# VITA-Group/CV_A-FAN

Measured on AMD Instinct MI355X. Metric: images/sec (whole node) A-FAN K=5 train step, ResNet-18/CIFAR-10, higher is better.
Workload: dtype bf16; 1 GPU; resnet18 CIFAR-10-shape A-FAN K=5 bf16, batch 256/GPU, perturb_idx 6, internal layout nhwc, 1xMI355X per rank (BASELINE configs[1]); global_batch=256, parallelism=dp1, hipgraph=True, in_launch_batchnorm=True

## Files before the change

### cv_a-fan_amd/_lib.py

```python
import ctypes as C
import os

_HERE = os.path.dirname(os.path.abspath(__file__))
LIB_PATH = os.environ.get("AFAN_HIP_LIB") or os.path.join(_HERE, "libafan_hip.so")

AFAN_F32, AFAN_BF16 = 0, 1
AFAN_NCHW, AFAN_NHWC = 0, 1
_ERRORS = {-1: "AFAN_EDTYPE (unknown dtype code)", -2: "AFAN_EALIGN (misaligned pointer)",
           -3: "AFAN_ESHAPE (bad sizes)", -4: "AFAN_ENULL (required pointer is NULL)",
           -5: "AFAN_ELAYOUT (unknown layout code)"}

_p, _i, _l, _f = C.c_void_p, C.c_int, C.c_int64, C.c_float

SIGNATURES = {
    "afan_version": (_i, []),
    "afan_arch": (C.c_char_p, []),
    "afan_pgd_step": (_i, [_p, _p, _i, _p, _p, _l, _f, _f, _i, _p]),
    "afan_tensor_clamp": (_i, [_p, _p, _p, _l, _p]),
    "afan_norms_workspace_floats": (_l, [_l, _l]),
    "afan_pgd_step_norms": (_i, [_p, _p, _i, _p, _p, _l, _l, _f, _f, _i, _p, _p, _p, _p]),
    "afan_perturb_norms": (_i, [_p, _p, _l, _l, _p, _p, _p, _p]),
    "afan_axpy_noise": (_i, [_p, _p, _l, _f, _p, _p]),
    "afan_mix_feature": (_i, [_p, _p, _p, _l, _l, _l, _f, _i, _p]),
    "afan_mix_feature_nhwc": (_i, [_p, _p, _p, _l, _l, _l, _f, _i, _p]),
    "afan_lerp_points": (_i, [_p, _p, _p, _l, C.POINTER(_f), _i, _p]),
    "afan_lerp_mix": (_i, [_p, _p, _p, _l, _l, _l, C.POINTER(_f), _i, C.c_uint, _f, _i, _p]),
    "afan_head_max_classes": (_i, []),
    "afan_head_forward": (_i, [_p, _i, _l, _l, _l, _p, _p, _l, _p, _p, _p]),
    "afan_head_backward": (_i, [_p, _p, _p, _l, _l, _l, _l, _p, _i, _p, _p, _i, _p]),
    "afan_cross_entropy": (_i, [_p, _p, _l, _l, _p, _p, _p]),
    "afan_mix_w_workspace_floats": (_l, []),
    "afan_mix_w": (_i, [_p, _p, _p, _p, _i, _l, _p]),
    "afan_mix_w_backward": (_i, [_p, _i, _p, _p, _l, _p, _p, _i, _p]),
    "afan_bn_workspace_floats": (_l, [_l]),
    "afan_bn_acc_doubles": (_l, [_l]),
    "afan_bn_acc_supported": (_i, [_i, _l]),
    "afan_bn_set_running_updates": (_i, [_i]),
    "afan_bn_running_update": (_i, [_p, _l, C.c_double, _f, _f, _p, _p, _p, _p]),
    "afan_bn_running_update_batched": (_i, [_p, _p, _p, _p, _p, _p, _p, _p, _i, _p]),
    "afan_bn_train_forward_acc": (_i, [_p, _p, _p, _i, _l, _l, _l, _f, _f, _p, _p, _i, _p, _i, _p, _p, _p, _p, _i, _p]),
    "afan_bn_train_forward_acc_dual": (_i, [_p, _p, _p, _i, _l, _l, _l, _f, _f, _p, _p, _p, _p, _p, _p, _p, _f, _f, _p, _p, _p, _p,
                                            _p, _p, _p, _p]),
    "afan_bn_backward_acc": (_i, [_p, _p, _p, _p, _p, _i, _l, _l, _l, _p, _i, _p, _i, _p, _p, _i, _i, _p]),
    "afan_bn_stats": (_i, [_p, _i, _i, _l, _l, _l, _f, _f, _p, _p, _p, _p, _p, _p]),
    "afan_bn_train_forward": (_i, [_p, _p, _p, _i, _i, _l, _l, _l, _f, _f, _p, _p, _i, _p, _p, _p, _p, _p, _p]),
    "afan_bn_apply": (_i, [_p, _p, _p, _i, _i, _l, _l, _l, _p, _p, _p, _p, _i, _p, _p]),
    "afan_bn_backward": (_i, [_p, _p, _p, _p, _p, _i, _i, _l, _l, _l, _p, _p, _p, _i, _p, _p, _p, _i, _p, _l, _p]),
    "afan_conv_supported": (_i, [_l, _l, _i, _i]),
    "afan_conv_fwd_nhwc_bf16": (_i, [_p, _p, _p, _l, _l, _l, _l, _l, _i, _i, _i, _p, _p, _p, _i, _p]),
    "afan_conv_fwd_affine_nhwc_bf16": (_i, [_p, _p, _p, _l, _l, _l, _l, _l, _i, _i, _p, _p, _i, _p]),
    "afan_conv_fwd_affine_any_nhwc_bf16": (_i, [_p, _p, _p, _l, _l, _l, _l, _l, _i, _i, _p, _p, _i, _p]),
    "afan_conv_fwd_multi_nhwc_bf16": (_i, [_p, _p, _p, _i, _l, _l, _l, _l, _l, _p, _i, _p, _p, _p, _i, _p]),
    "afan_conv_fwd_tiles": (_l, [_l, _l, _l, _l, _l, _i, _i]),
# ... 79 lines not shown
    "afan_proposal_rows": (_i, [_p, _l, _p, _l, _p, _l, _p, _p, _p]),
    "afan_labels_limit": (_i, [_p, _l, _l, _p, _l, _p]),
    "afan_det_loss_bwd": (_i, [_p, _p, _p, _p, _p, _p, _l, _l, _l, _l, _l, _p, _p, _p]),
    "afan_roi_align_fwd": (_i, [_p, _p, _p, _i, _i, _l, _l, _l, _l, _i, _i, _f, _i, _p]),
    "afan_roi_align_bwd": (_i, [_p, _p, _p, _i, _i, _l, _l, _l, _l, _l, _i, _i, _f, _i, _p]),
    "afan_roi_align_bwd_workspace_bytes": (_l, [_l, _l, _l]),
    "afan_roi_align_bwd_ws": (_i, [_p, _p, _p, _i, _i, _l, _l, _l, _l, _l, _i, _i, _f, _i, _p, _p]),
    "afan_transpose_weights": (_i, [_p, _p, _p, _i, _l, _p]),
    "afan_sgd_step": (_i, [_p, _p, _p, _p, _l, _p, _f, _f, _f, _i, _p]),
    "afan_sgd_step_guarded": (_i, [_p, _p, _p, _p, _l, _p, _f, _f, _f, _i, _p, _p]),
    "afan_guarded_copy": (_i, [_p, _p, _l, _p, _p, _p]),
    "afan_occupy_cus": (_i, [_i, _i, _i, _p]),
    "afan_cast_bf16": (_i, [_p, _p, _l, _p]),
    "afan_pgd_init": (_i, [_p, _i, _p, _p, _p, _l, _p]),
    "afan_normalize_nchw": (_i, [_p, _p, _i, _i, _l, _l, _l, _p, _p, _p]),
    "afan_profile_enable": (_i, [_i]),
    "afan_profile_collect": (_i, [C.c_char_p, C.POINTER(_l), C.POINTER(C.c_double), C.POINTER(C.c_double),
                                  C.POINTER(C.c_double), _i]),
    "afan_profile_event_overhead": (_i, [_i, C.POINTER(_f), _p]),
    "afan_conv_trace": (_i, [_i]),
    "afan_conv_trace_read": (_i, [C.POINTER(_l), C.c_char_p, _i]),
}

_lib = None


class AfanLibraryError(RuntimeError):
    pass


def load():
    global _lib
    if _lib is not None:
        return _lib
    if not os.path.exists(LIB_PATH):
        raise AfanLibraryError(
            f"{LIB_PATH} is missing: build it with `python -c 'import __graft_entry__ as g; g.build()'` "
            "(or `make -C cv_a-fan_amd/csrc`). There is no CPU or PyTorch fallback for the A-FAN kernels.")
    lib = C.CDLL(LIB_PATH)
    for name, (res, args) in SIGNATURES.items():
        fn = getattr(lib, name)
        fn.restype = res
        fn.argtypes = args
    _lib = lib
    return lib


def check(rc, what):
    if rc == 0:
        return
    if rc < 0:
        raise AfanLibraryError(f"{what}: {_ERRORS.get(rc, rc)}")
    raise AfanLibraryError(f"{what}: HIP launch failed with hipError_t={rc}")
```

### cv_a-fan_amd/attack_algo.py

```python
import torch

from . import ops
from .resnet_s import _dense, _like_layout, dgrad_only, fused_criterion

__all__ = ["PGD", "tensor_clamp", "linfball_proj", "mix_feature", "get_sample_points", "last_norms"]

_last = {"l2": None, "linf": None}


def last_norms():
    return _last["l2"], _last["linf"]


def tensor_clamp(t, min, max, in_place=True):
    res = t if in_place else t.clone()
    ops.tensor_clamp_(res.data, min.contiguous(), max.contiguous())
    return res


def linfball_proj(center, radius, t, in_place=True):
    res = t if in_place else t.clone()
    zero = torch.zeros_like(res.data)
    ops.pgd_step_(res.data, zero, 0.0, x_clean=center.contiguous(), eps=float(radius), clip=True)
    return res


def PGD(x, loss_fn, y=None, model=None, steps=3, gamma=None, start_idx=1, layer_number=16, eps=(2 / 255),
        randinit=False, clip=False, with_norms=False, grad0=None):
    if x.device.type != "cuda":
        raise ops.AfanLibraryError("PGD: x must live on the MI355X (no CPU path in this build)")
    lp = getattr(model, "compute_dtype", torch.float32) == torch.bfloat16
    if grad0 is not None and (randinit or steps < 1):
        raise ValueError("grad0 is the gradient at x: not with randinit, and only when there is a first step")
    x, x_adv, shadow = ops.pgd_init(_dense(x.detach()), want_shadow=lp and grad0 is None and not randinit)
    if lp and shadow is None:
        shadow = torch.empty_like(x, dtype=torch.bfloat16)
    if randinit:
        u = _like_layout(torch.rand(x_adv.shape).to(x.device, non_blocking=True), x_adv)
        ops.axpy_noise_(x_adv, u, eps, shadow)
    l2 = linf = None
    loss_fn = fused_criterion(loss_fn, model)
    for t in range(steps):
        if t == 0 and grad0 is not None:
            grad = grad0.detach()
        else:
            xin = (shadow if lp else x_adv).detach().requires_grad_(True)
            with dgrad_only():
                out = model(xin, end_point=layer_number, start_point=start_idx)
                loss = loss_fn(out, y)
                root = ops.one(loss.device) if (loss.dim() == 0 and loss.dtype == torch.float32) else None
                grad = torch.autograd.grad(loss, xin, grad_outputs=root, only_inputs=True)[0]
        grad = _like_layout(grad, x_adv)
        if with_norms and t == steps - 1:
            l2, linf = ops.pgd_step_norms_(x_adv, grad, gamma, x, eps, clip, shadow)
        else:
            ops.pgd_step_(x_adv, grad, gamma, x, eps, clip, shadow)
    if with_norms:
        if l2 is None:
            l2, linf = ops.perturb_norms(x_adv, x)
        _last["l2"], _last["linf"] = l2, linf
    x_adv.requires_grad_(True)
    if lp:
        x_adv._afan_shadow = shadow
    return x_adv


def mix_feature(clean_feature, adv_feature):
    return ops.mix_feature(_dense(clean_feature), _dense(adv_feature), 1e-5)


# ... 14 lines not shown
```

### cv_a-fan_amd/csrc/afan_bn_nhwc.hip

```cpp
#include "afan_common.h"
#include <stdlib.h>

using namespace afan;

namespace afan_nhwc {

constexpr int BLOCK = 256;
constexpr int MAX_G = 512;

template <typename T, int VEC> struct LdV {
    __device__ static __forceinline__ void ld(const T* p, float (&v)[VEC]) {
        if constexpr (VEC == 1) v[0] = Elt<T>::ld(p); else Elt<T>::ldv(p, v);
    }
    __device__ static __forceinline__ void st(T* p, const float (&v)[VEC]) {
        if constexpr (VEC == 1) Elt<T>::st(p, v[0]); else Elt<T>::stv(p, v);
    }
};

template <int VEC>
__device__ __forceinline__ void ld_coef(const float* __restrict__ p, int c0, float (&v)[VEC]) {
    if constexpr (VEC % 4 == 0) {
#pragma unroll
        for (int q = 0; q < VEC / 4; ++q) {
            const f32x4 t = *reinterpret_cast<const f32x4*>(p + c0 + 4 * q);
// ... 961 lines not shown
    return dtype == AFAN_F32 ? stats_only<float>(x, M, C, eps, mom, ws, stats_out, rm, rv, nbt, st)
                             : stats_only<uint16_t>(x, M, C, eps, mom, ws, stats_out, rm, rv, nbt, st);
}
int bwd(int dtype, const void* dy, const void* x, const void* y, void* dx, void* dres, int64_t M, int64_t C,
        const float* stats_in, int relu, float* ws, float* dw, float* db, int acc, hipStream_t st,
        const float* partials, int64_t partials_g) {
    return dtype == AFAN_F32
               ? backward<float>(dy, x, y, dx, dres, M, C, stats_in, relu, ws, dw, db, acc, st, partials, partials_g)
               : backward<uint16_t>(dy, x, y, dx, dres, M, C, stats_in, relu, ws, dw, db, acc, st, partials, partials_g);
}
int coefs(int64_t C, const float* mean, const float* invstd, const float* w, const float* b, float* out, hipStream_t st) {
    AFAN_PROF("bn_nhwc_coef_kernel", 24.0 * C, st);
    coef_kernel<<<(unsigned)((C + BLOCK - 1) / BLOCK), BLOCK, 0, st>>>((int)C, mean, invstd, w, b, out);
    AFAN_LAUNCH_CHECK();
    return AFAN_OK;
}
int set_running_updates(int n) {
    const int old = g_running_updates;
    g_running_updates = n < 0 ? 1 : n;
    return old;
}
int64_t workspace_floats(int64_t c) { return c > 0 ? 2 * c * MAX_G + 2 * c + 4 * c : 0; }

}
```

### cv_a-fan_amd/ops.py

```python
import ctypes as C
import os
import threading

import torch

from . import _lib
from ._lib import AFAN_BF16, AFAN_F32, AFAN_NCHW, AFAN_NHWC, AfanLibraryError, check

_DT = {torch.float32: AFAN_F32, torch.bfloat16: AFAN_BF16}
_ws_cache = {}
_tls = threading.local()
CALLS = {"conv_fwd": 0, "conv_dgrad": 0, "conv_wgrad": 0, "conv_general": 0, "vendor_conv": 0, "conv_bn_fused": 0}


def _need(t, name, dtype=None):
    if not isinstance(t, torch.Tensor):
        raise TypeError(f"{name}: expected a torch.Tensor")
    if t.device.type != "cuda":
        raise AfanLibraryError(f"{name}: tensor is on '{t.device}'. The A-FAN kernels are MI355X-only; "
                               "there is no CPU path (the CPU restatement under oracle/ is test infrastructure).")
    if not _dense(t):
        raise ValueError(f"{name}: tensor must be dense (contiguous NCHW or channels_last)")
    if dtype is not None and t.dtype != dtype:
        raise TypeError(f"{name}: expected {dtype}, got {t.dtype}")
    return t


def _dense(t):
    return t.is_contiguous() or (t.dim() == 4 and t.is_contiguous(memory_format=torch.channels_last))


def layout_of(t):
    if t.dim() == 4 and not t.is_contiguous() and t.is_contiguous(memory_format=torch.channels_last):
        return AFAN_NHWC
    return AFAN_NCHW
# ... 373 lines not shown
def head_forward(x, weight, bias):
    lib = _lib.load()
    _need(x, "x"), _need(weight, "weight", torch.float32)
    if x.dim() != 4 or not (layout_of(x) == AFAN_NHWC or x.shape[2] * x.shape[3] == 1) or x.dtype not in _DT:
        raise ValueError("head_forward: x must be a channels-last fp32/bf16 feature map")
    n, c, hw = _nchw(x)
    k = weight.shape[0]
    pooled = torch.empty(n, c, dtype=torch.float32, device=x.device)
    logits = torch.empty(n, k, dtype=torch.float32, device=x.device)
    check(lib.afan_head_forward(_ptr(x), _DT[x.dtype], n, c, hw, _ptr(weight), _ptr(bias), k, _ptr(pooled), _ptr(logits),
                                _stream(x)), "afan_head_forward")
    return logits, pooled


def head_backward(dlogits, weight, pooled, x_like, want_dx, dweight=None, dbias=None, accumulate=False):
    lib = _lib.load()
    _need(dlogits, "dlogits", torch.float32), _need(pooled, "pooled", torch.float32)
    n, c, hw = _nchw(x_like)
    dx = torch.empty_like(x_like) if want_dx else None
    check(lib.afan_head_backward(_ptr(dlogits.contiguous()), _ptr(weight), _ptr(pooled), n, c, hw, weight.shape[0], _ptr(dx),
                                 _DT[x_like.dtype], _ptr(dweight), _ptr(dbias), int(bool(accumulate)), _stream(x_like)),
          "afan_head_backward")
    return dx


def bn_stats(x, eps=1e-5, momentum=0.1, running_mean=None, running_var=None, num_batches=None):
    lib = _lib.load()
    _need(x, "x")
    n, c, hw = _nchw(x)
    stats = torch.empty(4, c, dtype=torch.float32, device=x.device)
    ws = _workspace(x, lib.afan_bn_workspace_floats(c), "bn")
    check(lib.afan_bn_stats(_ptr(x), _DT[x.dtype], layout_of(x), n, c, hw, float(eps), float(momentum), _ptr(ws),
                            _ptr(stats), _ptr(running_mean), _ptr(running_var), _ptr(num_batches), _stream(x)),
          "afan_bn_stats")
    return stats[0], stats[1]


class record_bn_updates:

    def __enter__(self):
        self.old = getattr(_tls, "bn_rec", None)
        self.items = _tls.bn_rec = []
        return self

    def __exit__(self, *exc):
        _tls.bn_rec = self.old
# ... 1380 lines not shown
```

### cv_a-fan_amd/resnet_s.py

```python
import contextlib
import os

import torch
import torch.nn as nn
import torch.nn.functional as F

from . import ops

__all__ = ["ResNet", "ResNet50", "BasicBlock", "Bottleneck", "resnet20", "resnet56", "resnet18", "resnet50", "ARCHS",
           "dgrad_only"]


class _Flags:
    param_grads = True
    weight_epoch = 0
    block_fusion = True
    wgrad_stash = False
    bn_groups = 1
    bn_branch = "main"


@contextlib.contextmanager
def dgrad_only():
    old = _Flags.param_grads
    _Flags.param_grads = False
    try:
        yield
    finally:
        _Flags.param_grads = old


@contextlib.contextmanager
def bn_groups(g):
    old = _Flags.bn_groups
    _Flags.bn_groups = int(g)
    try:
        yield
    finally:
        _Flags.bn_groups = old


def enable_dual_bn(model):
    bns = [m for m in model.modules() if isinstance(m, BatchNorm2d)]
    for b in bns:
        b.enable_dual()
    model._dual_bns = bns
    return model


@contextlib.contextmanager
def bn_branch(model, branch):
    bns = getattr(model, "_dual_bns", None)
    if not bns:
        yield
        return
    old = _Flags.bn_branch
    for b in bns:
        b.select(branch)
    _Flags.bn_branch = branch
    try:
        yield
    finally:
# ... 513 lines not shown
    def _backward(ctx, gout):
        if not (_WgradBatch.ON and ctx.want_pgrad and _WgradBatch.pending is None):
            return _BlockFn._backward_impl(ctx, gout)
        _WgradBatch.pending = []
        try:
            out = _BlockFn._backward_impl(ctx, gout)
        except BaseException:
            _WgradBatch.pending = None
            raise
        _WgradBatch.flush()
        return out

    @staticmethod
    def _backward_impl(ctx, gout):
        x, rawsc, ssc, *saved = ctx.saved_tensors
        blk, pg, n, G = ctx.blk, ctx.want_pgrad, ctx.n, ctx.G
        chain = blk._chain()
        raws, acts, stats = saved[0::3], saved[1::3], saved[2::3]
        need_dx = ctx.needs_input_grad[0]
        g = lambda p: p.grad if pg else None
        out = acts[-1]
        pre, done = _BlockFn._handoff_check(ctx, gout)
        bl = chain[-1][1]
        if done is not None:
            d_raw, dres = done, gout
        else:
            gout = _like_layout(gout, out)
            d_raw, dres = _bn_bwd_g(gout, raws[-1], out, stats[-1], bl, True, True, pg, pre, G)
        c1 = chain[0][0]
        wt10 = getattr(c1, "_arena_wt10", None) if (_BlockFn.MULTI_SC and blk._sc_kind == "conv" and G == 1 and need_dx
                                                     and n >= 2) else None
        pair = None
        sc_done = getattr(gout, "_afan_sc_done", None) if done is not None else None
        r0 = raws[0]
        if wt10 is not None:
            pair = sc_done if sc_done is not None else torch.empty((2 * r0.shape[0],) + tuple(r0.shape[1:]), dtype=r0.dtype,
                                                                   device=r0.device, memory_format=torch.channels_last)
        for i in range(n - 1, 0, -1):
            c, bp = chain[i][0], chain[i - 1][1]
            fused = None
            if G == 1 and ops.GRID_BN and c.kernel_size[0] in (1, 3) and c.stride[0] == 1:
                fused = ops.conv_dgrad_bn(d_raw, c.lp_weight_t(), acts[i - 1].shape[2:], raws[i - 1], stats[i - 1], True,
                                          dweight=g(bp.weight), dbias=g(bp.bias), accumulate=pg,
                                          dx_out=pair[:r0.shape[0]] if (pair is not None and i == 1) else None, dilation=c.dilation[0])
            if fused is None:
                d_a, part = ops.conv_dgrad(d_raw, c.lp_weight_t(), acts[i - 1].shape[2:], c.stride[0],
                                           bn_bwd=(raws[i - 1], stats[i - 1], True), partials_buf=c._bwd_buf, groups=G,
                                           dilation=c.dilation[0])
# ... 352 lines not shown
                db = torch.empty_like(bias) if bias is not None else None
        dx = ops.head_backward(g.float().contiguous(), weight, pooled, x, ctx.needs_input_grad[0], dw, db, accumulate=direct)
        if direct:
            dw = db = None
        return dx, dw, db, None


class _CEFn(torch.autograd.Function):

    @staticmethod
    def forward(ctx, logits, target):
        loss, dlogits = ops.cross_entropy(logits, target)
        ctx.save_for_backward(dlogits)
        return loss.reshape(())

    @staticmethod
    def backward(ctx, g):
        (dlogits,) = ctx.saved_tensors
        if g.data_ptr() == ops.one(g.device).data_ptr():
            return dlogits, None
        return dlogits * g, None


_FUSED_CE = os.environ.get("AFAN_FUSED_CE", "1") != "0"


def fused_criterion(criterion, model):
    if not (_FUSED_CE and type(criterion) is nn.CrossEntropyLoss and criterion.weight is None and criterion.ignore_index == -100
            and criterion.reduction == "mean" and getattr(criterion, "label_smoothing", 0.0) == 0.0
            and getattr(model, "compute_dtype", torch.float32) == torch.bfloat16):
        return criterion

    def ce(out, y):
        if (out.is_cuda and out.dtype == torch.float32 and out.dim() == 2 and out.is_contiguous() and y.dtype == torch.int64
                and y.dim() == 1 and 0 < out.numel() <= ops.CE_MAX_ELEMS):
            return _CEFn.apply(out, y)
        return criterion(out, y)
    return ce


_FUSED_HEAD = os.environ.get("AFAN_FUSED_HEAD", "1") != "0"


def _head_ok(x, lin):
    return (_FUSED_HEAD and x.is_cuda and x.dim() == 4 and x.dtype in (torch.float32, torch.bfloat16) and lin.weight.dtype == torch.float32
            and (x.is_contiguous(memory_format=torch.channels_last) and not x.is_contiguous() or x.shape[2] * x.shape[3] == 1)
            and lin.out_features <= 16)


def _head_in(x):
    if x.is_cuda and x.dim() == 4 and x.is_contiguous() and x.shape[2] * x.shape[3] > 1 and x.shape[1] > 1:
        return x.contiguous(memory_format=torch.channels_last)
    return x


class _LinearFn(torch.autograd.Function):

    @staticmethod
    def forward(ctx, x, weight, bias, want_pgrad):
        x = x.contiguous()
# ... 91 lines not shown
                m.compute_dtype = dtype
            elif isinstance(m, NormalizeByChannelMeanStd):
                m.out_dtype = dtype
        return self

    def forward(self, x, end_point=34, start_point=0):
        layers = list(self.sequential_model[start_point:end_point])
        if self.channels_last and x.dim() == 4 and x.is_floating_point():
            x = x if x.is_contiguous(memory_format=torch.channels_last) else \
                x.contiguous(memory_format=torch.channels_last)
        i, n = 0, len(layers)
        while i < n:
            L = layers[i]
            if isinstance(L, BatchNorm2d):
                x = _to_compute(x, self.compute_dtype)
                if i + 1 < n and isinstance(layers[i + 1], nn.ReLU):
                    x = L.fused(x, None, True)
                    i += 2
                    continue
                x = L.fused(x)
            elif (isinstance(L, _HeadPool) and i + 2 < n and isinstance(layers[i + 1], nn.Flatten)
                  and isinstance(layers[i + 2], nn.Linear) and _head_ok(_head_in(x), layers[i + 2])):
                lin = layers[i + 2]
                x = _HeadFn.apply(_head_in(x), lin.weight, lin.bias, _Flags.param_grads)
                i += 3
                continue
            elif isinstance(L, nn.Linear):
                x = _linear(x.float(), L)
            else:
                x = L(x)
            i += 1
        return x


class ResNet50(ResNet):

    def __init__(self, num_classes=1000, blocks=(3, 4, 6, 3), init_weight=1):
        nn.Module.__init__(self)
        from .deeplab import MaxPool2d, StemConv
        self.all_layers = 9
        layers = [NormalizeByChannelMeanStd(mean=[0.485, 0.456, 0.406], std=[0.229, 0.224, 0.225]),
                  StemConv(3, 64, kernel_size=7, stride=2, padding=3, bias=False), BatchNorm2d(64), nn.ReLU(),
                  MaxPool2d(3, 2, 1)]
        in_planes = 64
        for stage, (planes, nb) in enumerate(zip((64, 128, 256, 512), blocks)):
            for b in range(nb):
                layers.append(Bottleneck(in_planes, planes, 2 if (stage > 0 and b == 0) else 1))
# ... 30 lines not shown
```

### cv_a-fan_amd/train_step.py

```python
import torch
import torch.distributed as dist

from . import ops
from .arena import ArenaSGD, ParamArena
from .attack_algo import PGD, last_norms
from .grid_guard import GuardedTrainer


def warmup_lr(step, optimizer, warm_up_steps=200, max_lr=0.1):
    lr = step * max_lr / (warm_up_steps - 1)
    lr = min(lr, max_lr)
    for p in optimizer.param_groups:
        p["lr"] = lr
    return lr


class GradAllReducer:

    def __init__(self, arena, n_chunks=4, group=None):
        self.arena, self.group = arena, group
        self.world = dist.get_world_size(group) if dist.is_initialized() else 1
        self.chunks = _cut_chunks(arena, n_chunks)
        self.on_cuda = arena.grad.device.type == "cuda"
        self.stream = torch.cuda.Stream(device=arena.grad.device) if self.on_cuda else None
# ... 232 lines not shown
            key = tuple(inp.shape)
            if self._fold_auto.get(key) is None:
                self._fold_auto[key] = self._feature_elems(inp) >= self.FOLD_MIN_ELEMS
            return self._fold_auto[key]
        return True

    def _feature_elems(self, inp):
        m = self.model
        c, h, w = inp.shape[1], inp.shape[2], inp.shape[3]
        for mod in m.sequential_model[:self.perturb_idx]:
            c, h, w = _out_shape(mod, c, h, w)
        return inp.shape[0] * c * h * w

    def _forward_backward_folded(self, inp, target, overlap_allreduce):
        from . import ops, resnet_s
        m, idx, ln = self.model, self.perturb_idx, self.layer_number
        ops.acc_reset(inp.device)
        self.optimizer.zero_grad()
        crit = resnet_s.fused_criterion(self.criterion, m)
        half = ops.half(inp.device)
        with ops.bn_running_updates(2):
            fm_clean = m(inp, end_point=idx, start_point=0)
        xin = fm_clean.detach().requires_grad_(True)
        with ops.record_bn_updates() as clean_bn:
            output_clean = m(xin, end_point=ln, start_point=idx)
        loss_clean = crit(output_clean, target)
        with resnet_s.stash_wgrad():
            torch.autograd.backward(loss_clean, grad_tensors=half)
        g0 = xin.grad
        feature_map = fm_clean.detach()
        feature_map = feature_map.float() if feature_map.dtype != torch.float32 else feature_map
        feature_map_adv = PGD(feature_map, self.criterion, y=target, model=m, steps=self.steps,
                              gamma=(self.gamma / 255), start_idx=idx, layer_number=ln, eps=(self.eps / 255),
                              randinit=False, clip=self.clip, with_norms=True, grad0=g0)
        l2, linf = last_norms()
        adv_in = getattr(feature_map_adv, "_afan_shadow", None)
        if adv_in is None:
            adv_in = feature_map_adv.detach()
        output_adv = m(adv_in, end_point=ln, start_point=idx)
        loss_adv = crit(output_adv, target)
        torch.autograd.backward(loss_adv, grad_tensors=half)
        resnet_s.flush_wgrad(m)
        clean_bn.replay()
        if overlap_allreduce:
            self.reducer.begin()
        fm_clean.backward(g0)
        with torch.no_grad():
            loss = (loss_adv + loss_clean) / 2
            prec1 = (output_clean.argmax(dim=1) == target).float().sum() * (100.0 / target.shape[0])
        return {"loss": loss.detach(), "loss_adv": loss_adv.detach(), "loss_clean": loss_clean.detach(),
                "prec1": prec1, "l2": l2, "linf": linf, "x_adv": feature_map_adv.detach(),
                "feature_map": feature_map, "out_clean": output_clean.detach()}

    def _tail_segments(self):
        m, idx, ln = self.model, self.perturb_idx, self.layer_number
        cuts = [idx]
        for i in range(idx + 1, ln):
            mod = m.sequential_model[i]
            if getattr(mod, "_sc_kind", "identity") != "identity":
                cuts.append(i)
        cuts.append(ln)
        return [(cuts[k], cuts[k + 1]) for k in range(len(cuts) - 1)]

    def _param_range(self, a, b):
        pre = tuple(f"sequential_model.{i}." for i in range(a, b))
        idxs = [i for i, n in enumerate(self.arena.names) if n.startswith(pre)]
        return (idxs[0], idxs[-1] + 1) if idxs else (0, 0)

    def _phases_folded(self, inp, target, out):
        from . import ops, resnet_s
        m, idx, ln = self.model, self.perturb_idx, self.layer_number
        segs = self._tail_segments()
        ops.acc_reset(inp.device)
        self.optimizer.zero_grad()
        crit = resnet_s.fused_criterion(self.criterion, m)
        half = ops.half(inp.device)

        def run_segments(x0):
            ins, outs, h = [x0], [], x0
            for k, (a, b) in enumerate(segs):
                o = m(h, end_point=b, start_point=a)
                outs.append(o)
                if k + 1 < len(segs):
                    h = o.detach().requires_grad_(True)
                    ins.append(h)
            return ins, outs

        with ops.bn_running_updates(2):
            fm_clean = m(inp, end_point=idx, start_point=0)
        xin = fm_clean.detach().requires_grad_(True)
        with ops.record_bn_updates() as clean_bn:
            c_ins, c_outs = run_segments(xin)
        loss_clean = crit(c_outs[-1], target)
        with resnet_s.stash_wgrad():
            torch.autograd.backward(loss_clean, grad_tensors=half)
            for k in range(len(segs) - 2, -1, -1):
                c_outs[k].backward(c_ins[k + 1].grad)
        g0 = xin.grad
        feature_map = fm_clean.detach()
        feature_map = feature_map.float() if feature_map.dtype != torch.float32 else feature_map
        feature_map_adv = PGD(feature_map, self.criterion, y=target, model=m, steps=self.steps,
                              gamma=(self.gamma / 255), start_idx=idx, layer_number=ln, eps=(self.eps / 255),
                              randinit=False, clip=self.clip, with_norms=True, grad0=g0)
        l2, linf = last_norms()
# ... 253 lines not shown
```

### include/afan_hip.h

```cpp
#ifndef AFAN_HIP_H
#define AFAN_HIP_H

#include <stdint.h>

#ifdef __cplusplus
extern "C" {
#endif

typedef void* afan_stream_t;

enum { AFAN_F32 = 0, AFAN_BF16 = 1 };

enum { AFAN_NCHW = 0, AFAN_NHWC = 1 };

enum {
    AFAN_OK = 0,
    AFAN_EDTYPE = -1,
    AFAN_EALIGN = -2,
    AFAN_ESHAPE = -3,
    AFAN_ENULL = -4,
    AFAN_ELAYOUT = -5
};

int afan_version(void);
// ... 269 lines not shown
int afan_det_loss_bwd(const float* g_ce, const float* g_sl1, const float* save, const int64_t* rows, const int64_t* gt_labels,
                      const int64_t* batch, int64_t S, int64_t B, int64_t C, int64_t K, int64_t R, float* d_logits, float* d_deltas,
                      afan_stream_t stream);
int afan_roi_align_fwd(const void* x, const float* rois, void* y, int dtype, int layout, int64_t num_rois, int64_t c, int64_t h,
                       int64_t w, int pooled_h, int pooled_w, float spatial_scale, int sampling_ratio, afan_stream_t stream);
int afan_roi_align_bwd(const void* dy, const float* rois, float* dx, int dtype, int layout, int64_t num_rois, int64_t n, int64_t c,
                       int64_t h, int64_t w, int pooled_h, int pooled_w, float spatial_scale, int sampling_ratio,
                       afan_stream_t stream);
int64_t afan_roi_align_bwd_workspace_bytes(int64_t num_rois, int64_t h, int64_t w);
int afan_roi_align_bwd_ws(const void* dy, const float* rois, float* dx, int dtype, int layout, int64_t num_rois, int64_t n, int64_t c,
                          int64_t h, int64_t w, int pooled_h, int pooled_w, float spatial_scale, int sampling_ratio, void* workspace,
                          afan_stream_t stream);

int afan_head_max_classes(void);
int afan_head_forward(const void* x, int dtype, int64_t n, int64_t c, int64_t hw, const float* weight, const float* bias,
                      int64_t k, float* pooled, float* logits, afan_stream_t stream);
int afan_head_backward(const float* dlogits, const float* weight, const float* pooled, int64_t n, int64_t c, int64_t hw,
                       int64_t k, void* dx, int dx_dtype, float* dweight, float* dbias, int accumulate,
                       afan_stream_t stream);

int afan_cross_entropy(const float* logits, const int64_t* target, int64_t n, int64_t k, float* loss, float* dlogits,
                       afan_stream_t stream);

int afan_transpose_weights(const void* src_arena, void* dst_arena, const int64_t* desc_dev, int n_desc,
                           int64_t total_tiles, afan_stream_t stream);

int afan_sgd_step(float* param, const float* grad, float* momentum_buf, uint16_t* shadow_bf16,
                  int64_t n, const float* lr_dev, float momentum, float weight_decay,
                  float grad_scale, int first_step, afan_stream_t stream);

int afan_sgd_step_guarded(float* param, const float* grad, float* momentum_buf, uint16_t* shadow_bf16,
                          int64_t n, const float* lr_dev, float momentum, float weight_decay,
                          float grad_scale, int first_step, const void* guard, afan_stream_t stream);
int afan_guarded_copy(void* dst, const void* src, int64_t bytes, const void* guard, void* counter, afan_stream_t stream);
int afan_occupy_cus(int workgroups, int lds_bytes, int microseconds, afan_stream_t stream);

int afan_cast_bf16(const float* src, uint16_t* dst, int64_t n, afan_stream_t stream);
int afan_pgd_init(const void* x, int dtype, float* x32, float* x_adv, uint16_t* shadow, int64_t n, afan_stream_t stream);
int afan_normalize_nchw(const float* x, void* y, int out_dtype, int out_layout, int64_t n, int64_t c, int64_t hw,
                        const float* mean, const float* std, afan_stream_t stream);

int afan_profile_enable(int on);
int afan_profile_collect(char* names_out, int64_t* launches, double* total_ms, double* total_bytes,
                         double* total_flops, int max_kernels);
int afan_profile_event_overhead(int n, float* us_out, afan_stream_t stream);

// ... 8 lines not shown
```

Measured before the change: 33230 images/sec.

## Fuse network tail: avgpool, linear head, cross-entropy and last BN backward partials

Adds a single forward kernel that computes global average pooling, the linear head, softmax cross-entropy with its gradient, the broadcast pooled gradient and the BN-backward reduction partials of the final block, plus a matching backward apply kernel. Autograd wrappers route the head and CE through this path when a fused-CE criterion and target are supplied, in PGD steps and in both clean and adversarial passes. The goal is to cut several small launches and re-reads of the last feature map in each of the many forward/backward passes per A-FAN step. In exchange it adds a grid-wide last-block counter reduction, fragile tensor-identity checks on the gradient root, and eligibility limits (K≤16, C≤1024, bf16 NHWC).

```diff
diff --git a/cv_a-fan_amd/_lib.py b/cv_a-fan_amd/_lib.py
--- a/cv_a-fan_amd/_lib.py
+++ b/cv_a-fan_amd/_lib.py
@@ -29,6 +29,10 @@
     "afan_head_forward": (_i, [_p, _i, _l, _l, _l, _p, _p, _l, _p, _p, _p]),
     "afan_head_backward": (_i, [_p, _p, _p, _l, _l, _l, _l, _p, _i, _p, _p, _i, _p]),
     "afan_cross_entropy": (_i, [_p, _p, _l, _l, _p, _p, _p]),
+    "afan_tail_end_partials": (_l, [_i, _i, _l, _l, _l, _l]),
+    "afan_tail_end_workspace_floats": (_l, [_l]),
+    "afan_tail_end_forward": (_i, [_p, _p, _i, _i, _l, _l, _l, _p, _p, _p, _l, _p, _p, _p, _p, _p, _p, _p, _p, _p, _p, _p]),
+    "afan_tail_end_backward": (_i, [_p, _p, _p, _p, _p, _i, _i, _l, _l, _l, _p, _p, _p, _p, _i, _p, _l, _p]),
     "afan_mix_w_workspace_floats": (_l, []),
     "afan_mix_w": (_i, [_p, _p, _p, _p, _i, _l, _p]),
     "afan_mix_w_backward": (_i, [_p, _i, _p, _p, _l, _p, _p, _i, _p]),
@@ -154,6 +158,8 @@
     "afan_conv_trace_read": (_i, [C.POINTER(_l), C.c_char_p, _i]),
 }
 
+_NEWER = ("afan_tail_end_partials", "afan_tail_end_workspace_floats", "afan_tail_end_forward", "afan_tail_end_backward")
+
 _lib = None
 
 
@@ -171,11 +177,17 @@
             "(or `make -C cv_a-fan_amd/csrc`). There is no CPU or PyTorch fallback for the A-FAN kernels.")
     lib = C.CDLL(LIB_PATH)
     for name, (res, args) in SIGNATURES.items():
+        if name in _NEWER and os.environ.get("AFAN_HIP_LIB") and not hasattr(lib, name):
+            continue
         fn = getattr(lib, name)
         fn.restype = res
         fn.argtypes = args
     _lib = lib
     return lib
+
+
+def has(name):
+    return hasattr(load(), name)
 
 
 def check(rc, what):
diff --git a/cv_a-fan_amd/attack_algo.py b/cv_a-fan_amd/attack_algo.py
--- a/cv_a-fan_amd/attack_algo.py
+++ b/cv_a-fan_amd/attack_algo.py
@@ -1,7 +1,7 @@
 import torch
 
 from . import ops
-from .resnet_s import _dense, _like_layout, dgrad_only, fused_criterion
+from .resnet_s import _dense, _like_layout, dgrad_only, fused_criterion, tail_end
 
 __all__ = ["PGD", "tensor_clamp", "linfball_proj", "mix_feature", "get_sample_points", "last_norms"]
 
@@ -45,7 +45,7 @@
             grad = grad0.detach()
         else:
             xin = (shadow if lp else x_adv).detach().requires_grad_(True)
-            with dgrad_only():
+            with dgrad_only(), tail_end(y if getattr(loss_fn, "_afan_fused_ce", False) else None):
                 out = model(xin, end_point=layer_number, start_point=start_idx)
                 loss = loss_fn(out, y)
                 root = ops.one(loss.device) if (loss.dim() == 0 and loss.dtype == torch.float32) else None
diff --git a/cv_a-fan_amd/csrc/afan_bn_nhwc.hip b/cv_a-fan_amd/csrc/afan_bn_nhwc.hip
--- a/cv_a-fan_amd/csrc/afan_bn_nhwc.hip
+++ b/cv_a-fan_amd/csrc/afan_bn_nhwc.hip
@@ -1007,4 +1007,303 @@
 }
 int64_t workspace_floats(int64_t c) { return c > 0 ? 2 * c * MAX_G + 2 * c + 4 * c : 0; }
 
-}
+
+constexpr int TE_MAXK = 16;
+constexpr int TE_IMGS = 4;
+constexpr int TE_MAXC = 1024;
+
+__global__ __launch_bounds__(BLOCK) void tail_end_fwd_kernel(
+    const uint16_t* __restrict__ y, const uint16_t* __restrict__ x, const float* __restrict__ stats, const float* __restrict__ W,
+    const float* __restrict__ bias, const int64_t* __restrict__ target, const float* __restrict__ scale, float* __restrict__ pooled,
+    float* __restrict__ logits, float* __restrict__ loss, float* __restrict__ dlogits, float* __restrict__ dls,
+    uint16_t* __restrict__ grow, float* __restrict__ ws, float* lossrow, unsigned* counter, int N, int C, int HW, int K, int CV, int IPI) {
+    __shared__ float grp[TE_IMGS][BLOCK * 8];
+    __shared__ uint16_t gl[TE_IMGS][TE_MAXC];
+    __shared__ float red[TE_IMGS][BLOCK / AFAN_WAVE][TE_MAXK];
+    __shared__ float lg[TE_IMGS][TE_MAXK], ex[TE_IMGS][TE_MAXK], dl[TE_IMGS][TE_MAXK];
+    __shared__ int is_last;
+    const int tid = threadIdx.x, pc = tid % CV, pg = tid / CV, R = BLOCK / CV, G = gridDim.x;
+    const int64_t M = (int64_t)N * HW;
+    const int c0 = pc * 8, ITB = TE_IMGS / IPI;
+    const float inv = 1.0f / (float)HW, invn = 1.0f / (float)N;
+    const float sc = scale ? scale[0] : 1.f;
+    float mu[8];
+    ld_coef<8>(stats, c0, mu);
+    float acc[2][8];
+#pragma unroll
+    for (int k = 0; k < 8; ++k) acc[0][k] = acc[1][k] = 0.f;
+    for (int it0 = 0; ((int64_t)blockIdx.x + (int64_t)it0 * G) * R < M; it0 += ITB) {
+        int img[TE_IMGS];
+        bool ok[TE_IMGS], own[TE_IMGS];
+#pragma unroll
+        for (int s = 0; s < TE_IMGS; ++s) {
+            const int64_t row0 = ((int64_t)blockIdx.x + (int64_t)(it0 + s / IPI) * G) * R;
+            const int64_t im = row0 / HW + s % IPI;
+            ok[s] = row0 < M && im < N;
+            own[s] = ok[s] && row0 % HW == 0;
+            img[s] = ok[s] ? (int)im : 0;
+        }
+        float sa[TE_IMGS][8];
+#pragma unroll
+        for (int s = 0; s < TE_IMGS; ++s)
+#pragma unroll
+            for (int j = 0; j < 8; ++j) sa[s][j] = 0.f;
+        for (int p = pg; p < HW; p += R) {
+            u16x8 v[TE_IMGS];
+#pragma unroll
+            for (int s = 0; s < TE_IMGS; ++s)
+                if (ok[s]) v[s] = *reinterpret_cast<const u16x8*>(y + ((int64_t)img[s] * HW + p) * C + c0);
+#pragma unroll
+            for (int s = 0; s < TE_IMGS; ++s)
+                if (ok[s]) {
+#pragma unroll
+                    for (int j = 0; j < 8; ++j) sa[s][j] += bf2f(v[s][j]);
+                }
+        }
+#pragma unroll
+        for (int s = 0; s < TE_IMGS; ++s)
+#pragma unroll
+            for (int j = 0; j < 8; ++j) grp[s][pg * C + c0 + j] = sa[s][j];
+        __syncthreads();
+        float part[TE_IMGS][TE_MAXK];
+#pragma unroll
+        for (int s = 0; s < TE_IMGS; ++s)
+#pragma unroll
+            for (int k = 0; k < TE_MAXK; ++k) part[s][k] = 0.f;
+        for (int c = tid; c < C; c += BLOCK) {
+            float m[TE_IMGS];
+#pragma unroll
+            for (int s = 0; s < TE_IMGS; ++s) {
+                float t = 0.f;
+                for (int g = 0; g < R; ++g) t += grp[s][g * C + c];
+                m[s] = t * inv;
+                if (own[s]) pooled[(int64_t)img[s] * C + c] = m[s];
+            }
+#pragma unroll
+            for (int k = 0; k < TE_MAXK; ++k)
+                if (k < K) {
+                    const float w = W[(int64_t)k * C + c];
+#pragma unroll
+                    for (int s = 0; s < TE_IMGS; ++s) part[s][k] = fmaf(m[s], w, part[s][k]);
+                }
+        }
+#pragma unroll
+        for (int s = 0; s < TE_IMGS; ++s)
+#pragma unroll
+            for (int k = 0; k < TE_MAXK; ++k)
+                if (k < K) {
+                    const float v = wave_sum(part[s][k]);
+                    if ((tid & 63) == 0) red[s][tid >> 6][k] = v;
+                }
+        __syncthreads();
+        const int hs = (tid >> 4) & (TE_IMGS - 1), hk = tid & 15;
+        const bool head_t = tid < TE_IMGS * TE_MAXK && hk < K;
+        int h_img = 0;
+        bool h_own = false;
+#pragma unroll
+        for (int s = 0; s < TE_IMGS; ++s)
+            if (s == hs) { h_img = img[s]; h_own = own[s]; }
+        if (head_t) {
+            float t = bias ? bias[hk] : 0.f;
+            for (int w = 0; w < BLOCK / AFAN_WAVE; ++w) t += red[hs][w][hk];
+            lg[hs][hk] = t;
+            if (h_own) logits[(int64_t)h_img * K + hk] = t;
+        }
+        __syncthreads();
+        float mx = 0.f;
+        if (head_t) {
+            mx = lg[hs][0];
+            for (int k = 1; k < K; ++k) mx = fmaxf(mx, lg[hs][k]);
+            ex[hs][hk] = expf(lg[hs][hk] - mx);
+        }
+        __syncthreads();
+        if (head_t) {
+            float ssum = 0.f;
+            for (int k = 0; k < K; ++k) ssum += ex[hs][k];
+            const float lse = mx + logf(ssum);
+            const int64_t t64 = target[h_img];
+            const bool bad = t64 < 0 || t64 >= K;
+            const int t = bad ? 0 : (int)t64;
+            const float d = bad ? NAN : (expf(lg[hs][hk] - lse) - (hk == t ? 1.f : 0.f)) * invn;
+            const float dsc = scale ? d * sc : d;
+            dl[hs][hk] = dsc;
+            if (h_own) {
+                dlogits[(int64_t)h_img * K + hk] = d;
+                if (dls) dls[(int64_t)h_img * K + hk] = dsc;
+                if (hk == 0) __hip_atomic_store(lossrow + h_img, bad ? NAN : lse - lg[hs][t], __ATOMIC_RELAXED, __HIP_MEMORY_SCOPE_AGENT);
+            }
+        }
+        __syncthreads();
+        for (int c = tid; c < C; c += BLOCK) {
+            float g[TE_IMGS];
+#pragma unroll
+            for (int s = 0; s < TE_IMGS; ++s) g[s] = 0.f;
+            for (int k = 0; k < K; ++k) {
+                const float w = W[(int64_t)k * C + c];
+#pragma unroll
+                for (int s = 0; s < TE_IMGS; ++s) g[s] = fmaf(dl[s][k], w, g[s]);
+            }
+#pragma unroll
+            for (int s = 0; s < TE_IMGS; ++s) {
+                const uint16_t u = f2bf(g[s] * inv);
+                gl[s][c] = u;
+                if (own[s]) grow[(int64_t)img[s] * C + c] = u;
+            }
+        }
+        __syncthreads();
+        for (int si = 0; si < ITB; ++si) {
+            const int64_t row0 = ((int64_t)blockIdx.x + (int64_t)(it0 + si) * G) * R, row = row0 + pg;
+            if (row < M) {
+                const int slot = si * IPI + (int)(row / HW - row0 / HW);
+                float e[8], o[8];
+                LdV<uint16_t, 8>::ld(x + (row * CV + pc) * 8, e);
+                LdV<uint16_t, 8>::ld(y + (row * CV + pc) * 8, o);
+#pragma unroll
+                for (int k = 0; k < 8; ++k) {
+                    float g = bf2f(gl[slot][c0 + k]);
+                    g = (o[k] > 0.f) ? g : 0.f;
+                    acc[0][k] += g;
+                    acc[1][k] += g * (e[k] - mu[k]);
+                }
+            }
+        }
+        __syncthreads();
+    }
+    block_fold_store<8, 2, float>(acc, CV, C, G, ws);
+    asm volatile("s_waitcnt vmcnt(0)" ::: "memory");
+    __syncthreads();
+    if (tid == 0) {
+        const unsigned t = __hip_atomic_fetch_add(counter, 1u, __ATOMIC_RELAXED, __HIP_MEMORY_SCOPE_AGENT);
+        is_last = t + 1 == (unsigned)G;
+        if (is_last) __hip_atomic_store(counter, 0u, __ATOMIC_RELAXED, __HIP_MEMORY_SCOPE_AGENT);
+    }
+    __syncthreads();
+    if (!is_last) return;
+    float local = 0.f;
+    for (int r = tid; r < N; r += BLOCK) local += __hip_atomic_load(lossrow + r, __ATOMIC_RELAXED, __HIP_MEMORY_SCOPE_AGENT);
+    const float w = wave_sum(local);
+    float* lred = &red[0][0][0];
+    if ((tid & 63) == 0) lred[tid >> 6] = w;
+    __syncthreads();
+    if (tid == 0) {
+        float s = 0.f;
+        for (int i = 0; i < BLOCK / AFAN_WAVE; ++i) s += lred[i];
+        loss[0] = s * invn;
+    }
+}
+
+template <bool DRES>
+__global__ __launch_bounds__(BLOCK) void bwd_apply_bcast_kernel(const uint16_t* __restrict__ grow, const uint16_t* __restrict__ x,
+                                                                const uint16_t* __restrict__ y, uint16_t* __restrict__ dx,
+                                                                uint16_t* __restrict__ dres, int64_t nvec, int CV, int C, int HW,
+                                                                const float* __restrict__ stats, const float* __restrict__ coef) {
+    const int c0 = (threadIdx.x % CV) * 8;
+    float mu[8], alpha[8], B[8], D[8];
+    ld_coef<8>(stats, c0, mu);
+    ld_coef<8>(stats + 2 * C, c0, alpha);
+    ld_coef<8>(coef, c0, B);
+    ld_coef<8>(coef + C, c0, D);
+    const int64_t stride = (int64_t)gridDim.x * BLOCK;
+#pragma unroll 4
+    for (int64_t v = (int64_t)blockIdx.x * BLOCK + threadIdx.x; v < nvec; v += stride) {
+        const int img = (int)((unsigned)(v / CV) / (unsigned)HW);
+        float d[8], e[8], o[8];
+        LdV<uint16_t, 8>::ld(grow + (int64_t)img * C + c0, d);
+        LdV<uint16_t, 8>::ld(x + v * 8, e);
+        LdV<uint16_t, 8>::ld(y + v * 8, o);
+#pragma unroll
+        for (int k = 0; k < 8; ++k) {
+            const float g = (o[k] > 0.f) ? d[k] : 0.f;
+            d[k] = g;
+            e[k] = fmaf(g, alpha[k], fmaf(e[k] - mu[k], B[k], D[k]));
+        }
+        LdV<uint16_t, 8>::st(dx + v * 8, e);
+        if (DRES) LdV<uint16_t, 8>::st(dres + v * 8, d);
+    }
+}
+
+int64_t tail_end_plan(int dtype, int layout, int64_t n, int64_t c, int64_t hw, int64_t k, Plan* out = nullptr) {
+    if (dtype != AFAN_BF16 || layout != AFAN_NHWC) return 0;
+    if (n <= 0 || c <= 0 || hw <= 0 || k <= 0 || k > TE_MAXK || n * k > (1 << 16) || c > TE_MAXC || n * hw > 0x7FFFFFFF) return 0;
+    Plan p;
+    if (!make_plan<uint16_t>(n * hw, c, {}, p) || !p.vec) return 0;
+    const int64_t R = BLOCK / p.CV;
+    if (R <= hw ? hw % R != 0 : (R % hw != 0 || R / hw > TE_IMGS)) return 0;
+    if (out) *out = p;
+    return p.G;
+}
+
+int tail_end_fwd(const void* y, const void* x, const float* stats, const float* W, const float* bias, const int64_t* target,
+                 const float* scale, int64_t n, int64_t c, int64_t hw, int64_t k, float* pooled, float* logits, float* loss,
+                 float* dlogits, float* dls, void* grow, float* partials, float* lossrow, unsigned* counter, hipStream_t st) {
+    Plan p;
+    if (!tail_end_plan(AFAN_BF16, AFAN_NHWC, n, c, hw, k, &p)) return AFAN_ESHAPE;
+    for (const void* q : {y, x, (const void*)stats, (const void*)grow})
+        if (!aligned(q, 16)) return AFAN_ESHAPE;
+    const int R = BLOCK / p.CV, IPI = R > hw ? (int)(R / hw) : 1;
+    AFAN_PROF("tail_end_fwd_kernel", 2.0 * p.tensor_bytes, st);
+    tail_end_fwd_kernel<<<p.G, BLOCK, 0, st>>>((const uint16_t*)y, (const uint16_t*)x, stats, W, bias, target, scale, pooled, logits,
+                                                loss, dlogits, dls, (uint16_t*)grow, partials, lossrow, counter, (int)n, (int)c,
+                                                (int)hw, (int)k, p.CV, IPI);
+    AFAN_LAUNCH_CHECK();
+    return AFAN_OK;
+}
+
+int tail_end_bwd(const void* grow, const void* x, const void* y, void* dx, void* dres, int64_t n, int64_t c, int64_t hw,
+                 const float* stats, float* ws, float* dweight, float* dbias, int accumulate, const float* partials,
+                 int64_t partials_g, hipStream_t st) {
+    Plan p;
+    const int64_t M = n * hw;
+    if (M > 0x7FFFFFFF || !make_plan<uint16_t>(M, c, {grow, x, y, dx, dres}, p) || !p.vec || !aligned(stats, 16)) return AFAN_ESHAPE;
+    float* coef = ws + (int64_t)2 * c * MAX_G;
+    {
+        AFAN_PROF("bn_nhwc_finalize_kernel", 8.0 * c * partials_g, st);
+        finalize_kernel<uint16_t, 1><<<(unsigned)((c + 3) / 4), BLOCK, 0, st>>>(
+            partials, (int)partials_g, (int)c, nullptr, 1.0f / (float)M, (float)M, 0.f, 0.f, nullptr, nullptr, const_cast<float*>(stats),
+            coef, nullptr, nullptr, nullptr, dweight, dbias, accumulate, nullptr, 1);
+    }
+    AFAN_LAUNCH_CHECK();
+    const int grid = apply_grid(p, M * c);
+    AFAN_PROF("tail_end_bwd_apply_kernel", p.tensor_bytes * (3 + (dres ? 1 : 0)), st);
+    if (dres)
+        bwd_apply_bcast_kernel<true><<<grid, BLOCK, 0, st>>>((const uint16_t*)grow, (const uint16_t*)x, (const uint16_t*)y, (uint16_t*)dx,
+                                                            (uint16_t*)dres, p.nvec, p.CV, (int)c, (int)hw, stats, coef);
+    else
+        bwd_apply_bcast_kernel<false><<<grid, BLOCK, 0, st>>>((const uint16_t*)grow, (const uint16_t*)x, (const uint16_t*)y, (uint16_t*)dx,
+                                                             nullptr, p.nvec, p.CV, (int)c, (int)hw, stats, coef);
+    AFAN_LAUNCH_CHECK();
+    return AFAN_OK;
+}
+
+}
+
+extern "C" {
+
+int64_t afan_tail_end_partials(int dtype, int layout, int64_t n, int64_t c, int64_t hw, int64_t k) {
+    return afan_nhwc::tail_end_plan(dtype, layout, n, c, hw, k);
+}
+
+int afan_tail_end_forward(const void* y, const void* x, int dtype, int layout, int64_t n, int64_t c, int64_t hw, const float* stats,
+                          const float* weight, const float* bias, int64_t k, const int64_t* target, const float* scale, float* pooled,
+                          float* logits, float* loss, float* dlogits, float* dlogits_scaled, void* grow, float* partials,
+                          float* workspace, afan_stream_t stream) {
+    if (!afan_nhwc::tail_end_plan(dtype, layout, n, c, hw, k)) return AFAN_ESHAPE;
+    if (!y || !x || !stats || !weight || !target || !pooled || !logits || !loss || !dlogits || !grow || !partials || !workspace)
+        return AFAN_ENULL;
+    if ((scale != nullptr) != (dlogits_scaled != nullptr)) return AFAN_ENULL;
+    return afan_nhwc::tail_end_fwd(y, x, stats, weight, bias, target, scale, n, c, hw, k, pooled, logits, loss, dlogits, dlogits_scaled,
+                                   grow, partials, workspace + 4, reinterpret_cast<unsigned*>(workspace), (hipStream_t)stream);
+}
+
+int64_t afan_tail_end_workspace_floats(int64_t n) { return n > 0 ? 4 + n : 0; }
+
+int afan_tail_end_backward(const void* grow, const void* x, const void* y, void* dx, void* d_residual, int dtype, int layout, int64_t n,
+                           int64_t c, int64_t hw, const float* save_stats, float* workspace, float* dweight, float* dbias,
+                           int accumulate, const float* partials, int64_t partials_g, afan_stream_t stream) {
+    if (dtype != AFAN_BF16 || layout != AFAN_NHWC || n <= 0 || c <= 0 || hw <= 0 || partials_g <= 0) return AFAN_ESHAPE;
+    if (!grow || !x || !y || !dx || !save_stats || !workspace || !partials) return AFAN_ENULL;
+    return afan_nhwc::tail_end_bwd(grow, x, y, dx, d_residual, n, c, hw, save_stats, workspace, dweight, dbias, accumulate, partials,
+                                   partials_g, (hipStream_t)stream);
+}
+
+}
diff --git a/cv_a-fan_amd/ops.py b/cv_a-fan_amd/ops.py
--- a/cv_a-fan_amd/ops.py
+++ b/cv_a-fan_amd/ops.py
@@ -11,6 +11,7 @@
 _ws_cache = {}
 _tls = threading.local()
 CALLS = {"conv_fwd": 0, "conv_dgrad": 0, "conv_wgrad": 0, "conv_general": 0, "vendor_conv": 0, "conv_bn_fused": 0}
+TAIL_CALLS = {"fwd": 0, "bwd": 0}
 
 
 def _need(t, name, dtype=None):
@@ -430,6 +431,78 @@
                                  _DT[x_like.dtype], _ptr(dweight), _ptr(dbias), int(bool(accumulate)), _stream(x_like)),
           "afan_head_backward")
     return dx
+
+
+_te_ws = {}
+
+
+class TailEnd:
+    __slots__ = ("logits", "pooled", "loss", "dlogits", "dlogits_root", "grow", "partials", "g", "dy", "target", "scale", "armed")
+
+    fused = property(lambda self: self.grow is not None)
+
+
+def tail_end_forward(y, x, stats, weight, bias, target, scale=None, compose=True):
+    lib = _lib.load()
+    n, c, hw = _nchw(y)
+    k = weight.shape[0]
+    te = TailEnd()
+    te.target, te.scale, te.armed, te.grow, te.partials, te.g, te.dy = target, scale, False, None, None, 0, None
+    g = 0
+    if (_lib.has("afan_tail_end_forward") and y.is_cuda and y.dtype in _DT and y.dim() == 4 and x.shape == y.shape and x.dtype == y.dtype
+            and _dense(y) and _dense(x) and layout_of(x) == layout_of(y) and stats.dim() == 2 and stats.dtype == torch.float32
+            and stats.is_contiguous() and weight.dtype == torch.float32 and weight.is_contiguous() and weight.shape[1] == c
+            and (bias is None or (bias.dtype == torch.float32 and bias.is_contiguous()))
+            and target.is_cuda and target.dtype == torch.int64 and target.dim() == 1 and target.shape[0] == n and target.is_contiguous()
+            and (scale is None or (scale.is_cuda and scale.dtype == torch.float32 and scale.numel() == 1))):
+        g = int(lib.afan_tail_end_partials(_DT[y.dtype], layout_of(y), n, c, hw, k))
+    if g > 0:
+        dev = y.device
+        key = (dev.index, _raw_stream(dev.index))
+        ws = _te_ws.get(key)
+        need = int(lib.afan_tail_end_workspace_floats(n))
+        if ws is None or ws.numel() < need:
+            ws = _te_ws[key] = torch.zeros(max(need, 1024), dtype=torch.float32, device=dev)
+        te.pooled = torch.empty(n, c, dtype=torch.float32, device=dev)
+        te.logits = torch.empty(n, k, dtype=torch.float32, device=dev)
+        te.loss = torch.empty(1, dtype=torch.float32, device=dev)
+        te.dlogits = torch.empty(n, k, dtype=torch.float32, device=dev)
+        te.dlogits_root = torch.empty(n, k, dtype=torch.float32, device=dev) if scale is not None else te.dlogits
+        te.grow = torch.empty(n, c, dtype=y.dtype, device=dev)
+        te.partials = torch.empty(2 * c * g, dtype=torch.float32, device=dev)
+        te.g = g
+        rc = lib.afan_tail_end_forward(_ptr(y), _ptr(x), _DT[y.dtype], layout_of(y), n, c, hw, _ptr(stats), _ptr(weight), _ptr(bias), k,
+                                       _ptr(target), _ptr(scale), _ptr(te.pooled), _ptr(te.logits), _ptr(te.loss), _ptr(te.dlogits),
+                                       _ptr(te.dlogits_root) if scale is not None else None, _ptr(te.grow), _ptr(te.partials), _ptr(ws),
+                                       _stream(y))
+        if rc != -3:
+            check(rc, "afan_tail_end_forward")
+            TAIL_CALLS["fwd"] += 1
+            return te
+        te.grow, te.partials, te.g = None, None, 0
+    if not compose:
+        return None
+    te.logits, te.pooled = head_forward(y, weight, bias)
+    te.loss, te.dlogits = cross_entropy(te.logits, target)
+    te.dlogits_root = te.dlogits * scale if scale is not None else te.dlogits
+    te.dy = head_backward(te.dlogits_root, weight, te.pooled, y, True)
+    return te
+
+
+def tail_end_backward(te, x, y, stats, weight, bias, want_dres, dweight=None, dbias=None, accumulate=False):
+    if not te.fused:
+        return bn_backward(te.dy, x, y, stats, weight, bias, True, want_dres, dweight, dbias, accumulate)
+    lib = _lib.load()
+    n, c, hw = _nchw(x)
+    _same_layout(x, y)
+    dx = torch.empty_like(x)
+    dres = torch.empty_like(x) if want_dres else None
+    ws = _workspace(x, lib.afan_bn_workspace_floats(c), "bn")
+    check(lib.afan_tail_end_backward(_ptr(te.grow), _ptr(x), _ptr(y), _ptr(dx), _ptr(dres), _DT[x.dtype], layout_of(x), n, c, hw,
+                                     _ptr(stats), _ptr(ws), _ptr(dweight), _ptr(dbias), int(bool(accumulate)), _ptr(te.partials),
+                                     te.g, _stream(x)), "afan_tail_end_backward")
+    TAIL_CALLS["bwd"] += 1
+    return dx, dres
 
 
 def bn_stats(x, eps=1e-5, momentum=0.1, running_mean=None, running_var=None, num_batches=None):
diff --git a/cv_a-fan_amd/resnet_s.py b/cv_a-fan_amd/resnet_s.py
--- a/cv_a-fan_amd/resnet_s.py
+++ b/cv_a-fan_amd/resnet_s.py
@@ -18,6 +18,7 @@
     wgrad_stash = False
     bn_groups = 1
     bn_branch = "main"
+    tail_end = None
 
 
 @contextlib.contextmanager
@@ -38,6 +39,19 @@
         yield
     finally:
         _Flags.bn_groups = old
+
+
+_FUSED_TAILEND = os.environ.get("AFAN_FUSED_TAILEND", "1") != "0"
+
+
+@contextlib.contextmanager
+def tail_end(target, root=None):
+    old = _Flags.tail_end
+    _Flags.tail_end = (target, root) if (_FUSED_TAILEND and isinstance(target, torch.Tensor)) else None
+    try:
+        yield
+    finally:
+        _Flags.tail_end = old
 
 
 def enable_dual_bn(model):
@@ -597,8 +611,13 @@
         out = acts[-1]
         pre, done = _BlockFn._handoff_check(ctx, gout)
         bl = chain[-1][1]
+        te = getattr(gout, "_afan_tail", None) if (done is None and pre is None and G == 1) else None
+        if te is not None and getattr(gout, "_afan_tail_mark", None) != (gout.data_ptr(), gout._version, gout.stride()):
+            te = None
         if done is not None:
             d_raw, dres = done, gout
+        elif te is not None:
+            d_raw, dres = ops.tail_end_backward(te, raws[-1], out, stats[-1], bl.weight, bl.bias, True, g(bl.weight), g(bl.bias), pg)
         else:
             gout = _like_layout(gout, out)
             d_raw, dres = _bn_bwd_g(gout, raws[-1], out, stats[-1], bl, True, True, pg, pre, G)
@@ -997,6 +1016,78 @@
         return dlogits * g, None
 
 
+class _TailHeadFn(torch.autograd.Function):
+
+    @staticmethod
+    def forward(ctx, x, weight, bias, want_pgrad, te):
+        ctx.save_for_backward(x, weight, te.pooled)
+        ctx.bias, ctx.pg, ctx.te = bias, want_pgrad, te
+        logits, te.logits = te.logits, None
+        logits._afan_tail = te
+        return logits
+
+    @staticmethod
+    def backward(ctx, g):
+        x, weight, pooled = ctx.saved_tensors
+        bias, te = ctx.bias, ctx.te
+        want_p = ctx.pg and ctx.needs_input_grad[1]
+        dw = db = None
+        direct = False
+        if want_p:
+            direct = _accumulates_in_place(weight) and (bias is None or _accumulates_in_place(bias))
+            if direct:
+                dw, db = weight.grad, (bias.grad if bias is not None else None)
+            else:
+                dw = torch.empty_like(weight)
+                db = torch.empty_like(bias) if bias is not None else None
+        root = te.dlogits_root
+        fused = (te.armed and ctx.needs_input_grad[0] and g.dtype == torch.float32 and g.data_ptr() == root.data_ptr()
+                 and g.shape == root.shape and g.is_contiguous())
+        te.armed = False
+        if fused:
+            if want_p:
+                ops.head_backward(g, weight, pooled, x, False, dw, db, accumulate=direct)
+            dx = te.grow.view(x.shape[0], x.shape[1], 1, 1).expand(x.shape)
+            dx._afan_tail = te
+            dx._afan_tail_mark = (dx.data_ptr(), dx._version, dx.stride())
+        else:
+            dx = ops.head_backward(g.float().contiguous(), weight, pooled, x, ctx.needs_input_grad[0], dw, db, accumulate=direct)
+        if direct:
+            dw = db = None
+        return dx, dw, db, None, None
+
+
+class _TailCEFn(torch.autograd.Function):
+
+    @staticmethod
+    def forward(ctx, logits, te):
+        ctx.te = te
+        return te.loss.reshape(())
+
+    @staticmethod
+    def backward(ctx, g):
+        te = ctx.te
+        expect = te.scale if te.scale is not None else ops.one(g.device)
+        if g.dim() == 0 and g.dtype == torch.float32 and g.data_ptr() == expect.data_ptr():
+            te.armed = True
+            return te.dlogits_root, None
+        if g.data_ptr() == ops.one(g.device).data_ptr():
+            return te.dlogits, None
+        return te.dlogits * g, None
+
+
+def _tail_end_try(x, lin):
+    prev = getattr(x, "_afan_bn2", None)
+    if (prev is None or not _Flags.block_fusion or prev[2] != 1 or _Flags.bn_groups != 1 or not torch.is_grad_enabled()
+            or not x.requires_grad or x.dtype != torch.bfloat16):
+        return None
+    target, root = _Flags.tail_end
+    if not target.is_cuda or target.dim() != 1 or target.shape[0] != x.shape[0] or target.dtype != torch.int64:
+        return None
+    return ops.tail_end_forward(x, prev[0], prev[1], lin.weight.detach(), None if lin.bias is None else lin.bias.detach(),
+                                target.contiguous(), root, compose=False)
+
+
 _FUSED_CE = os.environ.get("AFAN_FUSED_CE", "1") != "0"
 
 
@@ -1007,10 +1098,14 @@
         return criterion
 
     def ce(out, y):
+        te = getattr(out, "_afan_tail", None)
+        if te is not None and isinstance(y, torch.Tensor) and y.data_ptr() == te.target.data_ptr() and y.shape == te.target.shape:
+            return _TailCEFn.apply(out, te)
         if (out.is_cuda and out.dtype == torch.float32 and out.dim() == 2 and out.is_contiguous() and y.dtype == torch.int64
                 and y.dim() == 1 and 0 < out.numel() <= ops.CE_MAX_ELEMS):
             return _CEFn.apply(out, y)
         return criterion(out, y)
+    ce._afan_fused_ce = True
     return ce
 
 
@@ -1148,7 +1243,12 @@
             elif (isinstance(L, _HeadPool) and i + 2 < n and isinstance(layers[i + 1], nn.Flatten)
                   and isinstance(layers[i + 2], nn.Linear) and _head_ok(_head_in(x), layers[i + 2])):
                 lin = layers[i + 2]
-                x = _HeadFn.apply(_head_in(x), lin.weight, lin.bias, _Flags.param_grads)
+                hx = _head_in(x)
+                te = _tail_end_try(hx, lin) if _Flags.tail_end is not None else None
+                if te is not None:
+                    x = _TailHeadFn.apply(hx, lin.weight, lin.bias, _Flags.param_grads, te)
+                else:
+                    x = _HeadFn.apply(hx, lin.weight, lin.bias, _Flags.param_grads)
                 i += 3
                 continue
             elif isinstance(L, nn.Linear):
diff --git a/cv_a-fan_amd/train_step.py b/cv_a-fan_amd/train_step.py
--- a/cv_a-fan_amd/train_step.py
+++ b/cv_a-fan_amd/train_step.py
@@ -278,7 +278,8 @@
         with ops.bn_running_updates(2):
             fm_clean = m(inp, end_point=idx, start_point=0)
         xin = fm_clean.detach().requires_grad_(True)
-        with ops.record_bn_updates() as clean_bn:
+        fused_ce = target if getattr(crit, "_afan_fused_ce", False) else None
+        with ops.record_bn_updates() as clean_bn, resnet_s.tail_end(fused_ce, half):
             output_clean = m(xin, end_point=ln, start_point=idx)
         loss_clean = crit(output_clean, target)
         with resnet_s.stash_wgrad():
@@ -293,7 +294,8 @@
         adv_in = getattr(feature_map_adv, "_afan_shadow", None)
         if adv_in is None:
             adv_in = feature_map_adv.detach()
-        output_adv = m(adv_in, end_point=ln, start_point=idx)
+        with resnet_s.tail_end(fused_ce, half):
+            output_adv = m(adv_in, end_point=ln, start_point=idx)
         loss_adv = crit(output_adv, target)
         torch.autograd.backward(loss_adv, grad_tensors=half)
         resnet_s.flush_wgrad(m)
@@ -335,7 +337,8 @@
         def run_segments(x0):
             ins, outs, h = [x0], [], x0
             for k, (a, b) in enumerate(segs):
-                o = m(h, end_point=b, start_point=a)
+                with resnet_s.tail_end(target if getattr(crit, "_afan_fused_ce", False) else None, half):
+                    o = m(h, end_point=b, start_point=a)
                 outs.append(o)
                 if k + 1 < len(segs):
                     h = o.detach().requires_grad_(True)
diff --git a/include/afan_hip.h b/include/afan_hip.h
--- a/include/afan_hip.h
+++ b/include/afan_hip.h
@@ -315,6 +315,16 @@
 int afan_cross_entropy(const float* logits, const int64_t* target, int64_t n, int64_t k, float* loss, float* dlogits,
                        afan_stream_t stream);
 
+int64_t afan_tail_end_partials(int dtype, int layout, int64_t n, int64_t c, int64_t hw, int64_t k);
+int64_t afan_tail_end_workspace_floats(int64_t n);
+int afan_tail_end_forward(const void* y, const void* x, int dtype, int layout, int64_t n, int64_t c, int64_t hw, const float* stats,
+                          const float* weight, const float* bias, int64_t k, const int64_t* target, const float* scale, float* pooled,
+                          float* logits, float* loss, float* dlogits, float* dlogits_scaled, void* grow, float* partials,
+                          float* workspace, afan_stream_t stream);
+int afan_tail_end_backward(const void* grow, const void* x, const void* y, void* dx, void* d_residual, int dtype, int layout, int64_t n,
+                           int64_t c, int64_t hw, const float* save_stats, float* workspace, float* dweight, float* dbias,
+                           int accumulate, const float* partials, int64_t partials_g, afan_stream_t stream);
+
 int afan_transpose_weights(const void* src_arena, void* dst_arena, const int64_t* desc_dev, int n_desc,
                            int64_t total_tiles, afan_stream_t stream);
 
```

Result: no change. 33010 images/sec (-0.7%).
